# Go2Heart/StreamFormer

Hardware: AMD Instinct MI355X
Metric: frames/s (16x224^2 clips) (higher is better)
Workload: dtype bf16; 1 GPU; SigLIP-base StreamFormer encoder forward, 8 clips x 16 x 224^2 per GPU, random-init de-trivialised weights, causal temporal attention; global_batch_clips=8, frames_per_clip=16, parallelism=dp1, steps_in_flight=1

## Files before the change

include/streamformer_hip.h:

```cpp
#ifndef STREAMFORMER_HIP_H
#define STREAMFORMER_HIP_H

#include <stddef.h>
#include <stdint.h>

#ifdef __cplusplus
extern "C" {
#endif

typedef struct sf_encoder sf_encoder;
typedef struct sf_cache sf_cache;
typedef void* sf_stream;

typedef enum {
  SF_OK = 0,
  SF_ERR_INVALID = -1,
  SF_ERR_STATE = -2,
  SF_ERR_HIP = -3,
  SF_ERR_WORKSPACE = -4,
  SF_ERR_UNKNOWN_KEY = -5,
  SF_ERR_CAPACITY = -6
} sf_status;

typedef enum { SF_F32 = 0, SF_BF16 = 1, SF_F16 = 2, SF_F64 = 3, SF_U8 = 4 } sf_dtype;
// ... 72 lines not shown
  int32_t H, W;
  int32_t layers, hidden_size, patches;
  int32_t elem_bytes;
  uint64_t packing;
  uint64_t blob_bytes;
} sf_cache_stream_meta;
int sf_cache_stream_blob_bytes(const sf_cache* cache, int stream, size_t* out);
int sf_cache_export_stream(sf_encoder* enc, sf_cache* cache, int stream, void* blob_dev, size_t bytes,
                           sf_cache_stream_meta* meta_out, sf_stream s);
int sf_cache_import_stream(sf_encoder* enc, sf_cache* cache, int stream, const void* blob_dev, size_t bytes,
                           const sf_cache_stream_meta* meta, sf_stream s);

int sf_op_layernorm(const float* x_dev, const float* gamma_dev, const float* beta_dev, float* y_dev,
                    int rows, int D, float eps, sf_stream stream);
int sf_op_linear(const float* x_dev, const float* w_dev, const float* b_dev, const float* resid_dev,
                 float alpha, int gelu, float* y_dev, int M, int N, int K, int compute,
                 void* workspace_dev, size_t workspace_bytes, sf_stream stream);
size_t sf_op_linear_workspace_bytes(int M, int N, int K);
typedef struct {
  int32_t split;
  const uint16_t* a_hi; const uint16_t* a_lo;
  const uint16_t* w_hi; const uint16_t* w_lo;
  const float* bias;
  int32_t M, N, K, epi, act;
  float alpha;
  const float* resid; int32_t resid_mod;
  const uint16_t* resid_hi; const uint16_t* resid_lo; const uint16_t* resid_lo2;
  const float* pos; const float* time_rows; int32_t Np, Tn;
  float* out_f32; uint16_t* out_hi; uint16_t* out_lo; uint16_t* out_lo2; int32_t ldc;
  int32_t grp_rows, grp_stride, grp_off;
  float* ln_stats_out; const float* ln_stats; const float* ln_s; float ln_eps; int32_t ln_stats_wide, ln_inkernel;
} sf_gemm_desc;
int sf_op_gemm(const sf_gemm_desc* d, int family, int* family_taken, sf_stream stream);
int sf_op_attention(const float* qkv_dev, float* ctx_dev, int groups, int L, int heads, int head_dim,
                    int causal, int temporal_layout, int N_tokens, int compute,
                    void* workspace_dev, size_t workspace_bytes, sf_stream stream);
size_t sf_op_attention_workspace_bytes(int groups, int L, int heads, int head_dim);
typedef struct { int32_t stream, t_row, slot, tk; } sf_stream_slot;
int sf_op_attention_cached(const float* cache_dev, float* ctx_dev, int slabs, int cap, int N_tokens, int heads, int head_dim,
                           int compute, int B, int Tq, int Tk, int q_t0, int t_past, int causal, const int* pos_dev,
                           const sf_stream_slot* tab_dev, int* route_out, int* waves_out,
                           void* workspace_dev, size_t workspace_bytes, sf_stream stream);
size_t sf_op_attention_cached_workspace_bytes(int slabs, int cap, int N_tokens, int heads, int head_dim, int B, int Tq);

size_t sf_loss_workspace_bytes(int B, int T);
int sf_retrieval_loss(const float* pooler_dev, const float* text_dev, int B, int T, int D, int Bt,
                      int pos_offset, const float* logit_scale_dev, const float* logit_bias_dev,
                      float* loss_dev, float* grad_pooler_dev, float* grad_scalars_dev,
                      void* workspace_dev, size_t workspace_bytes, sf_stream stream);
int sf_localization_loss(const float* pooler_dev, const float* label_emb_dev, const int32_t* labels_dev,
                         int B, int T, int D, int L, const float* logit_scale_dev, const float* logit_bias_dev,
                         float* loss_dev, float* grad_pooler_dev, float* grad_scalars_dev,
                         void* workspace_dev, size_t workspace_bytes, sf_stream stream);

int sf_grounding_loss(const float* pooler_dev, const float* text_dev, const float* labels_dev, int B, int T, int D,
                      const float* logit_scale_dev, const float* logit_bias_dev, float* loss_dev, float* grad_pooler_dev,
                      float* grad_scalars_dev, float* logits_out_dev, void* workspace_dev, size_t workspace_bytes,
                      sf_stream stream);
int sf_dense_text_logits(const float* x_dev, const float* text_dev, int M, int D, int n, const float* logit_scale_dev,
                         const float* logit_bias_dev, float* out_dev, sf_stream stream);

size_t sf_mask_loss_workspace_bytes(int B, int T, int N, int L_max);
int sf_mask_loss(const float* x_dev, int B, int T, int N, int D, const float* const* label_emb_dev,
                 const int32_t* num_labels, const int32_t* const* mask_dev, const int32_t* mask_width, int H,
                 const float* logit_scale_dev, const float* logit_bias_dev, float* loss_dev, float* grad_x_dev,
                 float* grad_scalars_dev, void* workspace_dev, size_t workspace_bytes, sf_stream stream);
// ... 292 lines not shown
```

streamformer_amd/_native.py:

```python
from __future__ import annotations

import ctypes as C
import inspect
import os
import weakref

import torch

_HERE = os.path.dirname(os.path.abspath(__file__))
LIB_PATH = os.path.join(_HERE, "libstreamformer_hip.so")
if os.environ.get("SF_LIB"):
    LIB_PATH = os.path.join(_HERE, "libstreamformer_hip_%s.so" % os.environ["SF_LIB"])

SF_OK = 0
SF_ERR_INVALID, SF_ERR_STATE, SF_ERR_HIP, SF_ERR_WORKSPACE, SF_ERR_UNKNOWN_KEY, SF_ERR_CAPACITY = -1, -2, -3, -4, -5, -6
SF_F32, SF_BF16, SF_F16, SF_F64, SF_U8 = 0, 1, 2, 3, 4
SF_COMPUTE_BF16, SF_COMPUTE_BF16X3 = 0, 1


class SfConfig(C.Structure):
    _fields_ = [(n, C.c_int32) for n in (
        "image_size", "patch_size", "num_channels", "num_frames", "hidden_size", "num_hidden_layers",
        "num_attention_heads", "intermediate_size", "hidden_act", "qkv_bias", "enable_causal_temporal",
        "add_lora_spatial")] + [("layer_norm_eps", C.c_float)]
# ... 68 lines not shown
    "sf_destroy": (None, [_P]),
    "sf_last_error": (C.c_char_p, []),
    "sf_abi_version": (_I, []),
    "sf_load_tensor": (_I, [_P, C.c_char_p, _P, _I, C.POINTER(C.c_int64), _I]),
    "sf_finalize_weights": (_I, [_P, _I, _I, _I]),
    "sf_missing_weights": (_I, [_P]),
    "sf_set_pixel_normalization": (_I, [_P, _P, _P, _I, _F]),
    "sf_workspace_bytes": (_I, [_P, _I, _I, _I, _I, C.POINTER(_SZ)]),
    "sf_forward": (_I, [_P, _P, _I, _I, _I, _I, _I, _P, _P, _P, _P, _P, _SZ, _P]),
    "sf_forward_profile": (_I, [_P, _P, _I, _I, _I, _I, _I, _P, _P, _P, _SZ, _P, C.POINTER(_F)]),
    "sf_forward_attentions": (_I, [_P, _P, _I, _I, _I, _I, _I, _P, _P, _P, _P, _P, _P, _SZ, _P]),
    "sf_embed": (_I, [_P, _P, _I, _I, _I, _I, _I, _P, _P, _P, _SZ, _P]),
    "sf_layers": (_I, [_P, _P, _I, _I, _I, _I, _I, _I, _P, _P, _SZ, _P]),
    "sf_post_head": (_I, [_P, _P, _I, _I, _I, _I, _P, _P, _P, _SZ, _P]),
    "sf_cache_create": (_I, [_P, _I, _I, _I, _I, C.POINTER(_P)]),
    "sf_cache_reset": (_I, [_P]),
    "sf_cache_length": (_I, [_P]),
    "sf_cache_stream_length": (_I, [_P, _I]),
    "sf_cache_reset_stream": (_I, [_P, _I]),
    "sf_cache_bytes": (_SZ, [_P]),
    "sf_cache_set_policy": (_I, [_P, _I]),
    "sf_cache_destroy": (None, [_P]),
    "sf_cache_stream_blob_bytes": (_I, [_P, _I, C.POINTER(_SZ)]),
    "sf_cache_export_stream": (_I, [_P, _P, _I, _P, _SZ, C.POINTER(SfCacheStreamMeta), _P]),
    "sf_cache_import_stream": (_I, [_P, _P, _I, _P, _SZ, C.POINTER(SfCacheStreamMeta), _P]),
    "sf_stream_workspace_bytes": (_I, [_P, _P, _I, C.POINTER(_SZ)]),
    "sf_forward_stream": (_I, [_P, _P, _P, _I, _I, _P, _P, _P, _P, _P, _SZ, _P]),
    "sf_forward_stream_slots": (_I, [_P, _P, _P, _I, _I, C.POINTER(_I), _I, _P, _P, _P, _P, _SZ, _P]),
    "sf_forward_stream_attentions": (_I, [_P, _P, _P, _I, _I, _P, _P, _P, _P, _P, _P, _SZ, _P]),
    "sf_op_layernorm": (_I, [_P, _P, _P, _P, _I, _I, _F, _P]),
    "sf_op_linear": (_I, [_P, _P, _P, _P, _F, _I, _P, _I, _I, _I, _I, _P, _SZ, _P]),
    "sf_op_linear_workspace_bytes": (_SZ, [_I, _I, _I]),
    "sf_op_gemm": (_I, [C.POINTER(SfGemmDesc), _I, C.POINTER(_I), _P]),
    "sf_op_attention": (_I, [_P, _P, _I, _I, _I, _I, _I, _I, _I, _I, _P, _SZ, _P]),
    "sf_op_attention_workspace_bytes": (_SZ, [_I, _I, _I, _I]),
    "sf_op_attention_cached": (_I, [_P, _P, _I, _I, _I, _I, _I, _I, _I, _I, _I, _I, _I, _I, _P, _P, C.POINTER(_I), C.POINTER(_I), _P, _SZ, _P]),
    "sf_op_attention_cached_workspace_bytes": (_SZ, [_I, _I, _I, _I, _I, _I, _I]),
    "sf_loss_workspace_bytes": (_SZ, [_I, _I]),
    "sf_retrieval_loss": (_I, [_P, _P, _I, _I, _I, _I, _I, _P, _P, _P, _P, _P, _P, _SZ, _P]),
    "sf_localization_loss": (_I, [_P, _P, _P, _I, _I, _I, _I, _P, _P, _P, _P, _P, _P, _SZ, _P]),
    "sf_grounding_loss": (_I, [_P, _P, _P, _I, _I, _I, _P, _P, _P, _P, _P, _P, _P, _SZ, _P]),
    "sf_dense_text_logits": (_I, [_P, _P, _I, _I, _I, _P, _P, _P, _P]),
    "sf_mask_loss_workspace_bytes": (_SZ, [_I, _I, _I, _I]),
    "sf_mask_loss": (_I, [_P, _I, _I, _I, _I, C.POINTER(_P), C.POINTER(C.c_int32), C.POINTER(_P), C.POINTER(C.c_int32), _I,
                          _P, _P, _P, _P, _P, _P, _SZ, _P]),
    "sf_dense_head_workspace_bytes": (_SZ, [_I, _I, _I]),
    "sf_dense_head_forward": (_I, [_P, _I, _I, _I, _F, C.POINTER(_P), _P, _P, _SZ, _P]),
    "sf_dense_head_backward": (_I, [_P, _I, _I, _I, _F, C.POINTER(_P), _P, C.POINTER(_P), _P, _SZ, _P]),
    "sf_trainer_create": (_I, [C.POINTER(SfConfig), _I, _I, _I, C.POINTER(_P)]),
    "sf_trainer_destroy": (None, [_P]),
    "sf_trainer_num_params": (_I, [_P]),
    "sf_trainer_param_info": (_I, [_P, _I, C.c_char_p, _I, C.POINTER(C.c_int64), C.POINTER(C.c_int64),
                                   C.POINTER(C.c_int64), C.POINTER(_I), C.POINTER(_I), C.POINTER(_I)]),
    "sf_trainer_total_floats": (_I, [_P, C.POINTER(C.c_int64), C.POINTER(C.c_int64)]),
    "sf_trainer_num_stages": (_I, [_P]),
    "sf_trainer_stage_range": (_I, [_P, _I, C.POINTER(C.c_int64), C.POINTER(C.c_int64)]),
    "sf_trainer_sync_weights": (_I, [_P, _P, _P]),
    "sf_trainer_workspace_bytes": (_I, [_P, _I, _I, C.POINTER(_SZ)]),
    "sf_trainer_forward": (_I, [_P, _P, _I, _I, _I, _P, _P, _P, _SZ, _P]),
    "sf_trainer_backward": (_I, [_P, _P, _P, _P, _I, _I, _P, _SZ, _P]),
    "sf_trainer_adamw_step": (_I, [_P, _P, _P, _P, _P, _I, _F, _F, _F, _F, _F, _F, _P, _F, _I, _P]),
    "sf_trainer_set_drop_path": (_I, [_P, _P, _I, _I]),
    "sf_trainer_set_dropout": (_I, [_P, _F, _F, C.c_uint32]),
    "sf_trainer_set_nonfinite_guard": (_I, [_P, _P, _P]),
    "sf_trainer_set_extra_steps": (_I, [_P, C.POINTER(C.c_int32), _I]),
    "sf_trainer_grad_sumsq": (_I, [_P, _P, _P, _P]),
# ... 259 lines not shown
```

streamformer_amd/csrc/sf_common.h:

```cpp
#pragma once
#include <hip/hip_runtime.h>
#include <stdint.h>

typedef unsigned short bf16_t;

typedef __attribute__((ext_vector_type(8))) short bf16x8_t;
typedef __attribute__((ext_vector_type(4))) float f32x4_t;
typedef __attribute__((ext_vector_type(4))) unsigned int u32x4_t;
typedef __attribute__((ext_vector_type(2))) unsigned int u32x2_t;

#define SF_DEVICE __device__ __forceinline__

#ifdef SF_LAB
#define SF_LAB_SWITCH(name) (getenv(name) ? atoi(getenv(name)) : 0)
#else
#define SF_LAB_SWITCH(name) 0
#endif

SF_DEVICE int sf_swz64(int row) {
#ifdef SF_SWZ64_LEGACY
  return (row >> 2) & 3;
#else
  return (0 - (row >> 2)) & 3;
#endif
// ... 162 lines not shown

struct __attribute__((aligned(16))) SfStreamSlot { int stream, t_row, slot, tk; };
#define SF_MAX_CALL_STREAMS 64
struct SfStreamTable { int n; int pad[3]; SfStreamSlot e[SF_MAX_CALL_STREAMS]; };

struct SfGemmArgs {
  const bf16_t* a_hi; const bf16_t* a_lo;
  const bf16_t* w_hi; const bf16_t* w_lo;
  const float* bias;
  int M, N, K;
  int epi;
  int act;
  float alpha;
  const float* resid;
  int resid_mod;
  const bf16_t* resid_hi; const bf16_t* resid_lo;
  const bf16_t* resid_lo2; bf16_t* out_lo2;
  const float* pos; const float* time_rows;
  int Np, Tn;
  const int* time_base_dev;
  float* out_f32;
  bf16_t* out_hi; bf16_t* out_lo;
  int ldc;
  int grp_rows, grp_stride, grp_off;
  const int* grp_off_dev; int grp_off_scale;
  const SfStreamSlot* grp_tab;
  int w_nt;
  float* ln_stats_out;
  const float* ln_stats; const float* ln_s; float ln_eps;
  int ln_stats_wide;
  int ln_inkernel;
  int aux_mode;
  bf16_t* aux;
};
SF_DEVICE size_t sf_out_row(const SfGemmArgs& p, int m) {
  if (p.grp_rows <= 0) return (size_t)m;
  if (p.grp_tab) {
    const int g = m / p.grp_rows;
    const SfStreamSlot e = p.grp_tab[g];
    return (size_t)e.stream * p.grp_stride + e.slot * p.grp_off_scale + (m - g * p.grp_rows);
  }
  const int off = p.grp_off + (p.grp_off_dev ? *p.grp_off_dev * p.grp_off_scale : 0);
  return (size_t)(m / p.grp_rows) * p.grp_stride + off + (m % p.grp_rows);
}
int sf_wall_clock_ticks(int ns);
enum SfGemmFamily {
  SF_GEMM_FAM_NONE = 0,
  SF_GEMM_FAM_SKINNY = 1, SF_GEMM_FAM_TILE = 2, SF_GEMM_FAM_PANEL = 3, SF_GEMM_FAM_G256 = 4, SF_GEMM_FAM_G128 = 5,
  SF_GEMM_FAM_COLSPLIT = 6,
  SF_GEMM_FAM_LAB_PIPE = 7, SF_GEMM_FAM_LAB_PP = 8,
};
SfGemmFamily sf_gemm_family(const SfGemmArgs& a, bool split);
hipError_t sf_launch_gemm_family(SfGemmFamily fam, const SfGemmArgs& a, bool split, hipStream_t s);
hipError_t sf_launch_gemm(const SfGemmArgs& a, bool split, hipStream_t s);
bool sf_gemm128_supported(const SfGemmArgs& a, bool split);
hipError_t sf_launch_gemm128(const SfGemmArgs& a, bool split, hipStream_t s);
bool sf_gemm256_supported(const SfGemmArgs& a, bool split);
bool sf_gemm256_aux_supported(const SfGemmArgs& a);
hipError_t sf_launch_gemm256(const SfGemmArgs& a, hipStream_t s);
int sf_skinny_max_rows();
bool sf_gemm_skinny_supported(const SfGemmArgs& a, bool split);
hipError_t sf_launch_gemm_skinny(const SfGemmArgs& a, bool split, hipStream_t s);
bool sf_gemm_tile_supported(const SfGemmArgs& a, bool split);
hipError_t sf_launch_gemm_tile(const SfGemmArgs& a, hipStream_t s);
int sf_tile_max_rows();
int sf_tile_fold_min_rows();
int sf_infold_max_rows();
struct SfQkvArgs {
  const bf16_t* a;
  const bf16_t* w;
  const float* bias; const float* ln_s;
  const float* ln_stats; float ln_eps;
  int M, K, D;
  int B, T, NP;
  bf16_t* out;
  float scale; int causal;
};
bool sf_gemm_qkv_supported(const SfQkvArgs& a, bool fused);
hipError_t sf_launch_gemm_qkv(const SfQkvArgs& a, bool fused, hipStream_t s);
struct SfStreamQkvArgs {
  const bf16_t* a;
  const bf16_t* w_frag;
  const float* bias; const float* ln_s; float ln_eps;
  int M, K, D, heads, N;
  bf16_t* cache;
  int cap, slot, Tk;
  const int* pos_dev;
  bf16_t* ctx;
  float scale;
};
bool sf_stream_qkv_decode_supported(const SfStreamQkvArgs& a);
hipError_t sf_launch_stream_qkv_decode(const SfStreamQkvArgs& a, hipStream_t s);
// ... 117 lines not shown
```

streamformer_amd/csrc/sf_gemm256.hip:

```cpp
#include "sf_common.h"
#include "sf_switches.h"
#include <cstdlib>

#define G_THREADS 512
#define PIECE_BYTES 16384

typedef const __attribute__((address_space(1))) void* gptr_t;
typedef __attribute__((address_space(3))) void* lptr_t;

SF_DEVICE f32x4_t mfma16b(bf16x8_t a, bf16x8_t b, f32x4_t c) {
  typedef __attribute__((ext_vector_type(8))) __bf16 v8bf;
  return __builtin_amdgcn_mfma_f32_16x16x32_bf16(__builtin_bit_cast(v8bf, a), __builtin_bit_cast(v8bf, b), c, 0, 0, 0);
}

SF_DEVICE bf16x8_t rd_frag(const char* piece, int row, int kc) {
  return *reinterpret_cast<const bf16x8_t*>(piece + row * 128 + ((kc ^ ((row >> 1) & 7)) << 4));
}
SF_DEVICE bf16x8_t rd_frag_s(const char* piece, int plane, int row, int g) {
  return *reinterpret_cast<const bf16x8_t*>(piece + plane * 8192 + row * 64 + ((g ^ sf_swz64(row)) << 4));
}

#ifdef SF_G256_TRACE
__device__ unsigned long long g256_trace[16];
#endif

template <int N>
SF_DEVICE void wait_vm() {
  asm volatile("s_waitcnt vmcnt(%0)" ::"n"(N) : "memory");
}

#define G256_EPI_BF16_AUX 5

template <int EPI, bool LNF, int BM, bool SPLIT = false, bool WIDE = false>
__global__ __launch_bounds__(G_THREADS) void sf_gemm256_kernel(SfGemmArgs p, int ntiles, int stagger_ticks, int stagger_groups) {
  constexpr int HR = BM / 2;
  constexpr int MT1 = (HR - 64) / 16;
  extern __shared__ __attribute__((aligned(16))) char smem[];
  const int tid = threadIdx.x;
  const int lane = tid & 63;
  const int wave = __builtin_amdgcn_readfirstlane(tid >> 6);
  const int wm = wave >> 2, wn = wave & 3;
  const int l15 = lane & 15, g = lane >> 4;
  const int tiles_n = p.N >> 8;
  const int K = p.K;
  const int nkt = SPLIT ? (K >> 5) : (K >> 6);
  const int dma_lds = wave * 1024;
  const __amdgpu_buffer_rsrc_t rsrc_a = __builtin_amdgcn_make_buffer_rsrc((void*)p.a_hi, 0, (unsigned)p.M * (unsigned)K * 2u, 0x00020000);
  const __amdgpu_buffer_rsrc_t rsrc_w = __builtin_amdgcn_make_buffer_rsrc((void*)p.w_hi, 0, (unsigned)p.N * (unsigned)K * 2u, 0x00020000);
  const __amdgpu_buffer_rsrc_t rsrc_al = __builtin_amdgcn_make_buffer_rsrc((void*)(SPLIT ? p.a_lo : p.a_hi), 0, (unsigned)p.M * (unsigned)K * 2u, 0x00020000);
  const __amdgpu_buffer_rsrc_t rsrc_wl = __builtin_amdgcn_make_buffer_rsrc((void*)(SPLIT ? p.w_lo : p.w_hi), 0, (unsigned)p.N * (unsigned)K * 2u, 0x00020000);
  const int cpx = gridDim.x >> 3;
  const int xcd = blockIdx.x & 7, slot_in_xcd = blockIdx.x >> 3;
  const int walk_cg = (stagger_groups >> 8) & 15;
  const bool store_wt = (stagger_groups >> 12) & 1;
  const bool store_nt = (stagger_groups >> 13) & 1;
  stagger_groups &= 255;
  const int walk_ngrp = walk_cg ? (tiles_n + walk_cg - 1) / walk_cg : 1;
  const int walk_per = (ntiles + 7) >> 3;
  const int walk_panels = ntiles / tiles_n;

  if (stagger_ticks > 0) {
    const int grp = slot_in_xcd % stagger_groups;
    if (grp) {
      const unsigned long long t0 = wall_clock64();
      const unsigned long long wait = (unsigned long long)grp * (unsigned long long)stagger_ticks;
      while (wall_clock64() - t0 < wait) __builtin_amdgcn_s_sleep(8);
    }
  }

#ifdef SF_G256_TRACE
  unsigned tr_read = 0, tr_bar1 = 0, tr_mma = 0, tr_bar2 = 0;
#endif
  for (int round = 0;; ++round) {
#ifdef SF_G256_TRACE
    tr_read = tr_bar1 = tr_mma = tr_bar2 = 0;
#endif
    int tile = (round * 8 + xcd) * cpx + slot_in_xcd;
    int m0, n0;
    if (walk_cg == 15) {
      const int sg = stagger_groups, grp = slot_in_xcd % sg, ig = slot_in_xcd / sg;
      const int n_g = (cpx - grp + sg - 1) / sg;
      const int before = grp * (cpx / sg) + min(grp, cpx % sg);
      const int x0 = xcd * walk_per, x1 = min(x0 + walk_per, ntiles);
      const int lo = x0 + (int)((long)(x1 - x0) * before / cpx), hi = x0 + (int)((long)(x1 - x0) * (before + n_g) / cpx);
      tile = lo + round * n_g + ig;
      if (tile >= hi) break;
      m0 = (tile / tiles_n) * BM; n0 = (tile % tiles_n) << 8;
    } else if (walk_cg) {
      const int tloc = round * cpx + slot_in_xcd;
      tile = xcd * walk_per + tloc;
      if (tloc >= walk_per || tile >= ntiles) break;
      int rest = tile, c0 = 0, w = 0;
      for (int j = 0; j < walk_ngrp; ++j) {
        w = tiles_n / walk_ngrp + (j < tiles_n % walk_ngrp ? 1 : 0);
        if (rest < walk_panels * w) break;
        rest -= walk_panels * w; c0 += w;
      }
      m0 = (rest / w) * BM; n0 = (c0 + rest % w) << 8;
    } else {
      if (tile >= ntiles) break;
      m0 = (tile / tiles_n) * BM; n0 = (tile % tiles_n) << 8;
    }

    unsigned offA[2][2], offB[2][2];
    int tid_p = threadIdx.x;
    asm volatile("" : "+v"(tid_p));
#pragma unroll
    for (int i = 0; i < (SPLIT ? 1 : 2); ++i) {
      const int c = i * G_THREADS + tid_p;
      const int prow = SPLIT ? (c >> 2) : (c >> 3), slot = SPLIT ? (c & 3) : (c & 7);
      const int kc = SPLIT ? (slot ^ sf_swz64(prow)) : (slot ^ ((prow >> 1) & 7));
#pragma unroll
      for (int q = 0; q < 2; ++q) {
        int rr = prow & 63;
        if (q == 1 && rr >= MT1 * 16) rr = MT1 * 16 - 1;
        int ar = m0 + (prow >> 6) * HR + q * 64 + rr;
        ar = ar < p.M ? ar : p.M - 1;
        offA[q][i] = ((unsigned)ar * (unsigned)K + kc * 8) * 2u;
        int br = n0 + (prow >> 5) * 64 + q * 32 + (prow & 31);
        offB[q][i] = ((unsigned)br * (unsigned)K + kc * 8) * 2u;
      }
    }
    auto issue = [&](int t, int j) {
      char* dst = smem + ((t & 1) * 4 + j) * PIECE_BYTES + dma_lds;
      const unsigned o0 = (j & 1) ? offA[j >> 1][0] : offB[j >> 1][0];
      const unsigned o1 = (j & 1) ? offA[j >> 1][SPLIT ? 0 : 1] : offB[j >> 1][SPLIT ? 0 : 1];
      const int kof = SPLIT ? t * 64 : t * 128;
      if (SPLIT) {
        if (j & 1) {
          __builtin_amdgcn_raw_ptr_buffer_load_lds(rsrc_a, (lptr_t)dst, 16, o0, kof, 0, 0);
          __builtin_amdgcn_raw_ptr_buffer_load_lds(rsrc_al, (lptr_t)(dst + 8192), 16, o1, kof, 0, 0);
        } else {
// ... 347 lines not shown
  if (split && a.ln_stats && (!a.ln_stats_wide || !a.ln_s || (a.K % 256) || a.K > 1024 || (a.epi != SF_EPI_BF16 && a.epi != SF_EPI_ACT_BF16))) return false;
  if (a.epi == SF_EPI_EMBED_F32) return false;
  bool planes = false;
  if (a.epi == SF_EPI_RESID_F32 && a.out_hi) {
    if (!a.out_lo || !a.resid_hi || !a.resid_lo || !a.ln_stats_out || !a.ln_stats_wide || (a.N % 256) || a.N > 1024 || a.grp_rows > 0) return false;
    if (!split && (a.resid_lo2 || a.out_lo2)) return false;
    planes = true;
  } else if (a.resid_hi) {
    return false;
  }
  if (!split && a.epi == SF_EPI_ACT_BF16 && a.act != 0 && a.act != 99) return false;
  if (a.K % 128 || a.K < 128) return false;
  int min_n = 1024;
  if (split) {
    min_n = a.M <= 6272 ? 1024 : 768;
    if (const char* e = sf_sw(SW_G256_SPLIT_MIN_N)) min_n = atoi(e);
  }
  if (a.N % 256 || a.N < min_n) return false;
  if (a.M < 2048 || (size_t)a.M * a.K * 2 >= ((size_t)1 << 32) || (size_t)a.N * a.K * 2 >= ((size_t)1 << 32)) return false;
  if (a.out_lo && !split && !planes) return false;
  return true;
}

bool sf_gemm256_aux_supported(const SfGemmArgs& a) {
  return a.epi == SF_EPI_BF16 && a.aux != nullptr && sf_gemm256_supported(a, false);
}

static int g256_grid() {
  int cus = sf_device_cus();
  if (cus < 8) cus = 256;
  return cus & ~7;
}

template <int BM, bool SPLIT_ONLY = false>
static hipError_t launch_bm(const SfGemmArgs& a_in, hipStream_t s) {
  SfGemmArgs a = a_in;
  if (SF_LAB_SWITCH("SF_G256_LAB_NOSTORE")) a.act = 99;
  const int tiles = ((a.M + BM - 1) / BM) * (a.N / 256);
  const size_t lds = 8 * PIECE_BYTES;
  const dim3 grid(g256_grid()), block(G_THREADS);
  int stagger = 0, sgroups = 3;
  if (const char* ge = sf_sw(SW_G256_STAGGER_GROUPS)) sgroups = atoi(ge) > 1 ? atoi(ge) : 2;
  {
    const int rounds = (tiles + (int)grid.x - 1) / (int)grid.x;
    double pct = 21.0;
    if (const char* pe = sf_sw(SW_G256_STAGGER_PCT)) pct = atof(pe);
    const char* env = sf_sw(SW_G256_STAGGER_NS);
    if (env) stagger = sf_wall_clock_ticks(atoi(env));
    else if (rounds >= 3) {
      const double mfma_x = (a.a_lo && a.w_lo) ? 3.0 : 1.0;
      const double tile_ns = mfma_x * 2.0 * BM * 256.0 * a.K / 3.9e3 + 6500.0;
      stagger = sf_wall_clock_ticks((int)(tile_ns * pct / 100.0));
    }
  }
  if (const char* only = sf_sw(SW_G256_STAGGER_ONLY)) {
    if (a.epi != atoi(only)) stagger = 0;
  }
  {
    int cg = 0;
    if (const char* we = sf_sw(SW_G256_WALK)) cg = atoi(we);
    if (cg < 0 || cg > 15 || (cg != 15 && cg >= a.N / 256)) cg = 0;
    sgroups = (sgroups & 255) | (cg << 8) | (sf_sw(SW_G256_STORE_WT) ? 1 << 12 : 0) | (sf_sw(SW_G256_STORE_NT) ? 1 << 13 : 0);
  }
#define SF_LAUNCH256(E, L, SP) return sf_launch_big_lds(sf_gemm256_kernel<E, L, BM, SP>, grid, block, lds, s, a, tiles, stagger, sgroups)
  if (a.a_lo && a.w_lo) {
    if (a.aux_mode) return hipErrorInvalidValue;
    if (a.ln_stats) {
      if (!a.ln_stats_wide || !a.ln_s) return hipErrorInvalidValue;
      if (a.epi == SF_EPI_BF16) SF_LAUNCH256(SF_EPI_BF16, true, true);
      if (a.epi == SF_EPI_ACT_BF16) SF_LAUNCH256(SF_EPI_ACT_BF16, true, true);
      return hipErrorInvalidValue;
    }
    switch (a.epi) {
#define SF_CASE(E) case E: SF_LAUNCH256(E, false, true);
      SF_CASE(SF_EPI_F32) SF_CASE(SF_EPI_BF16) SF_CASE(SF_EPI_ACT_BF16) SF_CASE(SF_EPI_RESID_F32)
#undef SF_CASE
      default: return hipErrorInvalidValue;
    }
  }
  if constexpr (SPLIT_ONLY) return hipErrorInvalidValue;
  else {
  const bool lnf = a.ln_stats != nullptr;
  if (lnf && (!a.ln_s || (a.epi != SF_EPI_BF16 && a.epi != SF_EPI_ACT_BF16))) return hipErrorInvalidValue;
  switch (a.epi) {
    case SF_EPI_F32: SF_LAUNCH256(SF_EPI_F32, false, false);
    case SF_EPI_BF16:
      if (a.aux_mode) {
        if (lnf || !a.aux) return hipErrorInvalidValue;
        SF_LAUNCH256(G256_EPI_BF16_AUX, false, false);
      }
      if (lnf) SF_LAUNCH256(SF_EPI_BF16, true, false);
      SF_LAUNCH256(SF_EPI_BF16, false, false);
    case SF_EPI_ACT_BF16:
      if (lnf) SF_LAUNCH256(SF_EPI_ACT_BF16, true, false);
      SF_LAUNCH256(SF_EPI_ACT_BF16, false, false);
    case SF_EPI_RESID_F32: SF_LAUNCH256(SF_EPI_RESID_F32, false, false);
    default: return hipErrorInvalidValue;
  }
  }
#undef SF_LAUNCH256
}

hipError_t sf_launch_gemm256(const SfGemmArgs& a, hipStream_t s) {
  const int g = g256_grid(), nt = a.N / 256;
  auto cost = [&](int bm) { const int tiles = ((a.M + bm - 1) / bm) * nt; return (long)((tiles + g - 1) / g) * bm; };
  if (a.a_lo && a.w_lo && !sf_sw(SW_G256_NO_SHORT_BM)) {
    auto t = [&](int bm, double f) { return (double)cost(bm) / bm * f; };
    const double t256 = t(256, 1632), t224 = t(224, 1472), t192 = t(192, 1370), t160 = t(160, 1268);
    const double best = fmin(fmin(t256, t224), fmin(t192, t160));
    if (const char* fe = sf_sw(SW_G256_FORCE_BM)) {
      switch (atoi(fe)) { case 160: return launch_bm<160, true>(a, s); case 192: return launch_bm<192, true>(a, s); case 224: return launch_bm<224>(a, s); default: return launch_bm<256>(a, s); }
    }
    if (best == t160 && t160 < 0.97 * fmin(t224, t256)) return launch_bm<160, true>(a, s);
    if (best == t192 && t192 < 0.97 * fmin(t224, t256)) return launch_bm<192, true>(a, s);
  }
  if (cost(224) < cost(256) && !sf_sw(SW_G256_NO_BM224)) return launch_bm<224>(a, s);
  return launch_bm<256>(a, s);
}
```

streamformer_amd/csrc/sf_ops.hip:

```cpp
#include "sf_handle.h"

#include <cmath>
#include <cstring>

__global__ void sf_combine_kernel(const bf16_t* hi, const bf16_t* lo, float* out, size_t n) {
  for (size_t i = (size_t)blockIdx.x * blockDim.x + threadIdx.x; i < n; i += (size_t)gridDim.x * blockDim.x)
    out[i] = bf2f(hi[i]) + (lo ? bf2f(lo[i]) : 0.f);
}

extern "C" int sf_op_layernorm(const float* x, const float* gamma, const float* beta, float* y, int rows, int D,
                               float eps, sf_stream stream) {
  HIP_TRY(sf_launch_layernorm(x, gamma, beta, y, nullptr, nullptr, rows, D, eps, (hipStream_t)stream));
  return SF_OK;
}

extern "C" size_t sf_op_linear_workspace_bytes(int M, int N, int K) {
  return ((size_t)M * K * 2 + (size_t)N * K * 2 + (size_t)M * N * 2) * 2 + 4096;
}

extern "C" int sf_op_linear(const float* x, const float* w, const float* b, const float* resid, float alpha, int gelu,
                            float* y, int M, int N, int K, int compute, void* workspace, size_t workspace_bytes,
                            sf_stream stream) {
  if (workspace_bytes < sf_op_linear_workspace_bytes(M, N, K)) return sf_set_err(SF_ERR_WORKSPACE, "workspace too small");
  hipStream_t s = (hipStream_t)stream;
  const bool split = compute == SF_COMPUTE_BF16X3;
  SfCarver c(workspace, split, true);
  const SfPlanes xp = c.planes((size_t)M * K), wp = c.planes((size_t)N * K), op = c.planes((size_t)M * N);
  HIP_TRY(sf_launch_split(x, xp.hi, xp.lo, (size_t)M * K, s));
  HIP_TRY(sf_launch_split(w, wp.hi, wp.lo, (size_t)N * K, s));
  SfGemmArgs g;
  memset(&g, 0, sizeof(g));
  g.a_hi = xp.hi; g.a_lo = xp.lo; g.w_hi = wp.hi; g.w_lo = wp.lo; g.bias = b;
  g.M = M; g.N = N; g.K = K; g.ldc = N; g.alpha = alpha; g.resid = resid; g.act = 0;
  if (gelu) {
    g.epi = SF_EPI_ACT_BF16; g.out_hi = op.hi; g.out_lo = op.lo;
    HIP_TRY(sf_launch_gemm(g, split, s));
    HIP_TRY(sf_launch(sf_combine_kernel, dim3(1024), dim3(256), 0, s, op.hi, op.lo, y, (size_t)M * N));
  } else {
    g.epi = resid ? SF_EPI_RESID_F32 : SF_EPI_F32; g.out_f32 = y;
    HIP_TRY(sf_launch_gemm(g, split, s));
  }
  return SF_OK;
}

static const char* gemm_family_name(int f) {
  static const char* const names[] = {"none", "skinny", "tile", "panel", "256^2", "128^2", "256-column + 128-column tail", "lab pipe", "lab pp"};
  return f >= 0 && f <= 8 ? names[f] : "?";
}
extern "C" int sf_op_gemm(const sf_gemm_desc* d, int family, int* family_taken, sf_stream stream) {
  if (family_taken) *family_taken = SF_GEMM_FAM_NONE;
  if (!d) return sf_set_err(SF_ERR_INVALID, "sf_op_gemm: null descriptor");
  if (family < 0 || family > SF_GEMM_FAM_G128) return sf_set_err(SF_ERR_INVALID, "sf_op_gemm: family %d is not one of 0 (dispatch) .. 5", family);
  const bool split = d->split != 0;
  if (d->M <= 0 || d->N <= 0 || d->K <= 0) return sf_set_err(SF_ERR_INVALID, "sf_op_gemm: bad shape M=%d N=%d K=%d", d->M, d->N, d->K);
  if (d->ldc < d->N) return sf_set_err(SF_ERR_INVALID, "sf_op_gemm: ldc %d < N %d", d->ldc, d->N);
  if (!d->a_hi || !d->w_hi) return sf_set_err(SF_ERR_INVALID, "sf_op_gemm: a_hi and w_hi are required");
  if (split && (!d->a_lo || !d->w_lo)) return sf_set_err(SF_ERR_INVALID, "sf_op_gemm: split needs a_lo and w_lo");
  if (!split && (d->a_lo || d->w_lo)) return sf_set_err(SF_ERR_INVALID, "sf_op_gemm: a_lo / w_lo given without split");
  if (d->act < 0 || d->act > 2) return sf_set_err(SF_ERR_INVALID, "sf_op_gemm: act %d is not 0 (erf GELU), 1 (tanh GELU) or 2 (ReLU)", d->act);
  if (d->resid_mod < 0) return sf_set_err(SF_ERR_INVALID, "sf_op_gemm: resid_mod %d < 0", d->resid_mod);
  if (d->resid_mod > 0 && !d->resid) return sf_set_err(SF_ERR_INVALID, "sf_op_gemm: resid_mod needs the fp32 resid table");
  if ((d->resid_hi != nullptr) != (d->resid_lo != nullptr)) return sf_set_err(SF_ERR_INVALID, "sf_op_gemm: resid_hi and resid_lo come together");
  if (d->resid_lo2 && !d->resid_hi) return sf_set_err(SF_ERR_INVALID, "sf_op_gemm: resid_lo2 needs resid_hi and resid_lo");
  if (d->resid && d->resid_hi) return sf_set_err(SF_ERR_INVALID, "sf_op_gemm: resid and resid_hi / resid_lo are two forms of one operand: give one");
  if (d->out_lo && !d->out_hi) return sf_set_err(SF_ERR_INVALID, "sf_op_gemm: out_lo needs out_hi");
  if (d->out_lo2 && !d->out_lo) return sf_set_err(SF_ERR_INVALID, "sf_op_gemm: out_lo2 needs out_hi and out_lo");
  if (!d->ln_inkernel && (d->ln_stats != nullptr) != (d->ln_s != nullptr))
    return sf_set_err(SF_ERR_INVALID, "sf_op_gemm: ln_stats and ln_s come together");
  if (d->ln_inkernel && !d->ln_s) return sf_set_err(SF_ERR_INVALID, "sf_op_gemm: ln_inkernel needs ln_s");
  if (d->ln_inkernel && d->ln_stats) return sf_set_err(SF_ERR_INVALID, "sf_op_gemm: ln_inkernel and ln_stats are two forms of one fold: give one");
  if ((d->ln_stats || d->ln_inkernel) && d->ln_stats_out) return sf_set_err(SF_ERR_INVALID, "sf_op_gemm: a fold consumer does not produce statistics");
  if (d->grp_rows < 0 || (d->grp_rows > 0 && (d->grp_stride < d->grp_rows || d->grp_off < 0)))
    return sf_set_err(SF_ERR_INVALID, "sf_op_gemm: row remap grp_rows=%d grp_stride=%d grp_off=%d (stride >= rows > 0, off >= 0)", d->grp_rows, d->grp_stride, d->grp_off);
  switch (d->epi) {
// ... 187 lines not shown
```

streamformer_amd/csrc/sf_switches.h:

```cpp
#pragma once

#define SF_SWITCH_TABLE(X) \
  X(ACC_TWO_PLANES, "SF_ACC_TWO_PLANES", "accurate mode: residual stream as two planes instead of three (A/B; max-abs 1.4e-4 instead of 5e-5)") \
  X(ASSUME_CUS, "SF_ASSUME_CUS", "size persistent grids for this many CUs (CU-masked stream experiments)") \
  X(DISABLE_ACC_FOLD, "SF_DISABLE_ACC_FOLD", "accurate mode: fp32 residual + standalone LayerNorm instead of the folded plane form (A/B)") \
  X(DISABLE_G256_SPLIT, "SF_DISABLE_G256_SPLIT", "accurate mode: keep the bf16x3 GEMMs off the persistent 256-column kernel") \
  X(DISABLE_GEMM_COLSPLIT, "SF_DISABLE_GEMM_COLSPLIT", "N = 256 j + 128 (so400m widths): the whole GEMM on 128^2 tiles instead of 256-column kernel + a 128-column tail (A/B)") \
  X(DISABLE_GEMM_MID, "SF_DISABLE_GEMM_MID", "skinny family: no 64 x 64 tiles above 512 rows") \
  X(DISABLE_GEMM_TILE, "SF_DISABLE_GEMM_TILE", "one / two clips per call: no tile-GEMM family") \
  X(DISABLE_LN_FOLD, "SF_DISABLE_LN_FOLD", "bf16 mode: standalone LayerNorm launches instead of the fold into the consumer GEMMs (A/B)") \
  X(DISABLE_RESID_PLANES, "SF_DISABLE_RESID_PLANES", "bf16 mode: fp32 residual stream instead of hi + lo planes (A/B)") \
  X(DISABLE_SKG_UNROLL, "SF_DISABLE_SKG_UNROLL", "streaming: K-parallel skinny GEMM with a run-time K-tile count (A/B)") \
  X(DISABLE_SKINNY, "SF_DISABLE_SKINNY", "send small-M GEMMs to the generic 128^2 kernel") \
  X(DISABLE_SPATIAL_DMA, "SF_DISABLE_SPATIAL_DMA", "spatial attention on the register-staged kernel") \
  X(DISABLE_SPATIAL_DMA_ACC, "SF_DISABLE_SPATIAL_DMA_ACC", "accurate mode: spatial attention on fp32 q / k / v (test coverage of that path)") \
  X(DISABLE_SPATIAL_NTC, "SF_DISABLE_SPATIAL_NTC", "spatial attention with a run-time tile count (A/B)") \
  X(DISABLE_STREAM_FOLD, "SF_DISABLE_STREAM_FOLD", "streaming: standalone LayerNorm launches (A/B)") \
  X(DISABLE_STREAM_GRAPH, "SF_DISABLE_STREAM_GRAPH", "streaming: eager launches instead of hipGraph replay") \
  X(DISABLE_TEMPORAL_DECODE, "SF_DISABLE_TEMPORAL_DECODE", "streaming: general temporal kernel instead of the single-query one") \
  X(TBWD_OWN_CU, "SF_TBWD_OWN_CU", "training: temporal attention backward as 12-wave workgroups that own a CU instead of 4-wave workgroups with their exact LDS (bit-identical, 65 against 51 us per launch; for jobs that share a device, DESIGN.md 4)") \
  X(TEMPORAL_DECODE_LANE_KEY, "SF_TEMPORAL_DECODE_LANE_KEY", "streaming: single-query temporal kernel with one key per lane (A/B against whole-line loads)") \
  X(DISABLE_TEMPORAL_DMA, "SF_DISABLE_TEMPORAL_DMA", "temporal attention on the register-staged kernel") \
  X(DISABLE_TEMPORAL_DMA_ACC, "SF_DISABLE_TEMPORAL_DMA_ACC", "accurate mode: temporal attention on fp32 q / k / v (test coverage of that path)") \
  X(EMBED_VIA_GEMM128, "SF_EMBED_VIA_GEMM128", "embedding GEMM on the generic kernel (A/B)") \
  X(G256_FORCE_BM, "SF_G256_FORCE_BM", "256-column kernel: force the row-tile height (tests of the short tiles)") \
  X(G256_NO_BM224, "SF_G256_NO_BM224", "256-column kernel: no 224-row tiles") \
  X(G256_NO_SHORT_BM, "SF_G256_NO_SHORT_BM", "256-column kernel, accurate mode: no 160 / 192-row tiles") \
  X(G256_SPLIT_MIN_N, "SF_G256_SPLIT_MIN_N", "accurate mode: smallest N the persistent kernel takes") \
  X(G256_WALK, "SF_G256_WALK", "256-column kernel: column-group width (tiles) of the column-group-major tile walk, 0 = row-major (A/B of the fabric traffic)") \
  X(G256_STORE_WT, "SF_G256_STORE_WT", "256-column kernel: bf16 outputs leave with write-through (sc1) stores that do not stay in the XCD's L2 (A/B)") \
  X(G256_STORE_NT, "SF_G256_STORE_NT", "256-column kernel: bf16 outputs leave with non-temporal stores (A/B: do the residual planes then survive in the Infinity Cache?)") \
  X(G256_STAGGER_GROUPS, "SF_G256_STAGGER_GROUPS", "256-column kernel: phase-stagger groups per XCD") \
  X(G256_STAGGER_NS, "SF_G256_STAGGER_NS", "256-column kernel: stagger step in ns (overrides the percentage)") \
  X(G256_STAGGER_ONLY, "SF_G256_STAGGER_ONLY", "256-column kernel: stagger only some launches (A/B)") \
  X(G256_STAGGER_PCT, "SF_G256_STAGGER_PCT", "256-column kernel: stagger step as a percentage of the tile period") \
  X(GEMM_MID_MIN_M, "SF_GEMM_MID_MIN_M", "skinny family: first M of the 64 x 64 tiles") \
  X(LN_BWD_BLOCKS, "SF_LN_BWD_BLOCKS", "LayerNorm backward: workgroups (tuning)") \
  X(POOL_SHARE_CU, "SF_POOL_SHARE_CU", "pooling head: the probe / combine kernels request only the LDS they use instead of a CU's whole 160 KB (A/B; with it other workgroups share their CUs, see DESIGN.md 4 on device sharing)") \
  X(PANEL_MIN_FILL_PCT, "SF_PANEL_MIN_FILL_PCT", "panel kernel: minimum last-round fill") \
  X(PANEL_PAD_CLAMP, "SF_PANEL_PAD_CLAMP", "panel kernel: clamp instead of zero-fill the padding rows (A/B)") \
  X(PANEL_STAGGER_NS, "SF_PANEL_STAGGER_NS", "panel kernel: phase-stagger step in ns") \
  X(SKINNY_MAX_M, "SF_SKINNY_MAX_M", "skinny family: largest M") \
  X(SKINNY_NO_KG, "SF_SKINNY_NO_KG", "skinny family: no K-parallel variant") \
  X(SKINNY_NB, "SF_SKINNY_NB", "streaming, folded skinny consumers: 1 = 32 x 32 tiles everywhere, 2 / 3 = force 32 x 64 / 32 x 96 tiles (A/B)") \
  X(SKINNY_NT, "SF_SKINNY_NT", "skinny family: non-temporal weight loads (A/B)") \
  X(SKINNY_TPS, "SF_SKINNY_TPS", "skinny family: tiles per slot (tuning)") \
  X(SPATIAL_PERS, "SF_SPATIAL_PERS", "lab library: persistent spatial attention kernel") \
  X(SPATIAL_TPW, "SF_SPATIAL_TPW", "spatial attention: query tiles per workgroup (tuning)") \
  X(STREAM_GRAPH_PER_POSITION, "SF_STREAM_GRAPH_PER_POSITION", "streaming: one graph per cache position instead of the position-free one (A/B)") \
  X(TILE_FOLD_MIN_M, "SF_TILE_FOLD_MIN_M", "tile-GEMM family: smallest M whose LayerNorm fold uses a statistics buffer and the 256^2 consumers") \
  X(TILE_MAX_M, "SF_TILE_MAX_M", "tile-GEMM family: largest M") \
  X(TILE_MIN_M, "SF_TILE_MIN_M", "tile-GEMM family: smallest M") \
  X(TILE_SHAPE, "SF_TILE_SHAPE", "tile-GEMM family: force a tile shape (tools/tile_lab.py)") \
  X(TRAIN_UNFUSED_TEMPORAL, "SF_TRAIN_UNFUSED_TEMPORAL", "training: temporal_attention.output.dense and temporal_dense as two launches instead of one fused projection (A/B)") \
  X(TRAIN_SIDE_STREAM, "SF_TRAIN_SIDE_STREAM", "training: 0 keeps the LoRA gradients on the caller stream (A/B)") \
  X(WGRAD_NSPLIT, "SF_WGRAD_NSPLIT", "weight-gradient GEMM: force the token splits") \
  X(WGRAD_SMALL_TILES, "SF_WGRAD_SMALL_TILES", "weight-gradient GEMM: 128^2 tiles only") \
  X(WGRAD_UNGROUPED, "SF_WGRAD_UNGROUPED", "training: one weight-gradient launch per projection instead of one per layer (test / A/B)") \

enum SfSw {
#define SF_SW_ENUM(id, name, what) SW_##id,
  SF_SWITCH_TABLE(SF_SW_ENUM)
// ... 5 lines not shown
```

Before: 15780 frames/s.

## Plan tail-round tile split across phase-staggered groups in the 256-column GEMM

Adds a host-side run planner that sizes each stagger group's tile share by when that group starts, so early-starting groups take more tail tiles and later groups fewer, rather than splitting in proportion to slot counts. The persistent 256-column kernel reads the planned group boundaries and, in the row-major walk, hands out last-round tiles per group from them. The aim is to shorten the tail left idle by the phase stagger. The cost is extra index arithmetic in the kernel and a planner whose timing model (tile period, step fraction) may not match the hardware.

```diff
diff --git a/include/streamformer_hip.h b/include/streamformer_hip.h
--- a/include/streamformer_hip.h
+++ b/include/streamformer_hip.h
@@ -128,6 +128,8 @@
   float* ln_stats_out; const float* ln_stats; const float* ln_s; float ln_eps; int32_t ln_stats_wide, ln_inkernel;
 } sf_gemm_desc;
 int sf_op_gemm(const sf_gemm_desc* d, int family, int* family_taken, sf_stream stream);
+int sf_g256_plan_runs(int tiles, int slots, int groups, double step, int* counts, double* ends);
+int sf_g256_launch_plan(int M, int N, int K, int split, int* out, double* ends);
 int sf_op_attention(const float* qkv_dev, float* ctx_dev, int groups, int L, int heads, int head_dim,
                     int causal, int temporal_layout, int N_tokens, int compute,
                     void* workspace_dev, size_t workspace_bytes, sf_stream stream);
diff --git a/streamformer_amd/_native.py b/streamformer_amd/_native.py
--- a/streamformer_amd/_native.py
+++ b/streamformer_amd/_native.py
@@ -124,6 +124,8 @@
     "sf_op_linear": (_I, [_P, _P, _P, _P, _F, _I, _P, _I, _I, _I, _I, _P, _SZ, _P]),
     "sf_op_linear_workspace_bytes": (_SZ, [_I, _I, _I]),
     "sf_op_gemm": (_I, [C.POINTER(SfGemmDesc), _I, C.POINTER(_I), _P]),
+    "sf_g256_plan_runs": (_I, [_I, _I, _I, C.c_double, C.POINTER(_I), C.POINTER(C.c_double)]),
+    "sf_g256_launch_plan": (_I, [_I, _I, _I, _I, C.POINTER(_I), C.POINTER(C.c_double)]),
     "sf_op_attention": (_I, [_P, _P, _I, _I, _I, _I, _I, _I, _I, _I, _P, _SZ, _P]),
     "sf_op_attention_workspace_bytes": (_SZ, [_I, _I, _I, _I]),
     "sf_op_attention_cached": (_I, [_P, _P, _I, _I, _I, _I, _I, _I, _I, _I, _I, _I, _I, _I, _P, _P, C.POINTER(_I), C.POINTER(_I), _P, _SZ, _P]),
diff --git a/streamformer_amd/csrc/sf_common.h b/streamformer_amd/csrc/sf_common.h
--- a/streamformer_amd/csrc/sf_common.h
+++ b/streamformer_amd/csrc/sf_common.h
@@ -218,6 +218,7 @@
   int ln_inkernel;
   int aux_mode;
   bf16_t* aux;
+  int g256_b1, g256_b2;
 };
 SF_DEVICE size_t sf_out_row(const SfGemmArgs& p, int m) {
   if (p.grp_rows <= 0) return (size_t)m;
@@ -244,6 +245,7 @@
 bool sf_gemm256_supported(const SfGemmArgs& a, bool split);
 bool sf_gemm256_aux_supported(const SfGemmArgs& a);
 hipError_t sf_launch_gemm256(const SfGemmArgs& a, hipStream_t s);
+void sf_gemm256_launch_plan(int M, int N, int K, bool split, int* out, double* ends);
 int sf_skinny_max_rows();
 bool sf_gemm_skinny_supported(const SfGemmArgs& a, bool split);
 hipError_t sf_launch_gemm_skinny(const SfGemmArgs& a, bool split, hipStream_t s);
diff --git a/streamformer_amd/csrc/sf_g256_plan.h b/streamformer_amd/csrc/sf_g256_plan.h
--- /dev/null
+++ b/streamformer_amd/csrc/sf_g256_plan.h
@@ -0,0 +1,82 @@
+#pragma once
+
+#define SF_G256_PLAN_MAX_GROUPS 8
+
+struct SfG256RunPlan {
+  int count[SF_G256_PLAN_MAX_GROUPS];
+  int slots[SF_G256_PLAN_MAX_GROUPS];
+  double end;
+  double end_proportional;
+  int weighted;
+};
+
+static inline int sf_g256_slots_before(int slots, int groups, int g) { return g * (slots / groups) + (g < slots % groups ? g : slots % groups); }
+
+static inline int sf_g256_proportional_bound(int tiles, int slots, int groups, int g) {
+  return (int)((long long)tiles * sf_g256_slots_before(slots, groups, g) / slots);
+}
+
+static inline double sf_g256_plan_end(const int* count, const int* slots, int groups, double step) {
+  double end = 0.0;
+  for (int g = 0; g < groups; ++g) {
+    if (count[g] <= 0) continue;
+    const double e = g * step + (double)((count[g] + slots[g] - 1) / slots[g]);
+    if (e > end) end = e;
+  }
+  return end;
+}
+
+static inline bool sf_g256_plan_group_runs(int tiles, int slots, int groups, double step, SfG256RunPlan* plan) {
+  if (tiles < 0 || slots < 1 || groups < 2 || groups > SF_G256_PLAN_MAX_GROUPS || groups > slots || !(step >= 0.0)) return false;
+  int prop[SF_G256_PLAN_MAX_GROUPS];
+  for (int g = 0; g < groups; ++g) {
+    plan->slots[g] = sf_g256_slots_before(slots, groups, g + 1) - sf_g256_slots_before(slots, groups, g);
+    prop[g] = sf_g256_proportional_bound(tiles, slots, groups, g + 1) - sf_g256_proportional_bound(tiles, slots, groups, g);
+  }
+  plan->end_proportional = sf_g256_plan_end(prop, plan->slots, groups, step);
+  const double eps = 1e-9;
+  const int max_rounds = (tiles + plan->slots[groups - 1] - 1) / plan->slots[groups - 1] + 1;
+  double best = -1.0;
+  for (int gc = 0; gc < groups; ++gc)
+    for (int r = 0; r <= max_rounds; ++r) {
+      const double e = gc * step + r;
+      if (best >= 0.0 && e >= best - eps) break;
+      long long cap = 0;
+      for (int g = 0; g < groups; ++g) {
+        const double room = e - g * step + eps;
+        if (room >= 1.0) cap += (long long)plan->slots[g] * (long long)room;
+      }
+      if (cap >= tiles) { best = e; break; }
+    }
+  if (best < 0.0 || best >= plan->end_proportional - eps) {
+    for (int g = 0; g < groups; ++g) plan->count[g] = prop[g];
+    plan->end = plan->end_proportional;
+    plan->weighted = 0;
+    return true;
+  }
+  long long slack = -(long long)tiles;
+  int rounds[SF_G256_PLAN_MAX_GROUPS];
+  for (int g = 0; g < groups; ++g) {
+    const double room = best - g * step + eps;
+    rounds[g] = room >= 1.0 ? (int)room : 0;
+    plan->count[g] = plan->slots[g] * rounds[g];
+    slack += plan->count[g];
+  }
+  while (slack > 0) {
+    int last = -1;
+    double last_end = -1.0;
+    for (int g = 0; g < groups; ++g) {
+      if (plan->count[g] <= 0) continue;
+      const double e = g * step + (double)((plan->count[g] + plan->slots[g] - 1) / plan->slots[g]);
+      if (e > last_end + eps) { last_end = e; last = g; }
+    }
+    const int spare = (plan->count[last] - 1) % plan->slots[last];
+    long long take = spare > 0 ? spare : 1;
+    if (take > slack) take = slack;
+    plan->count[last] -= (int)take;
+    slack -= take;
+  }
+  plan->end = sf_g256_plan_end(plan->count, plan->slots, groups, step);
+  plan->weighted = 1;
+  return true;
+}
diff --git a/streamformer_amd/csrc/sf_gemm256.hip b/streamformer_amd/csrc/sf_gemm256.hip
--- a/streamformer_amd/csrc/sf_gemm256.hip
+++ b/streamformer_amd/csrc/sf_gemm256.hip
@@ -1,5 +1,6 @@
 #include "sf_common.h"
 #include "sf_switches.h"
+#include "sf_g256_plan.h"
 #include <cstdlib>
 
 #define G_THREADS 512
@@ -54,6 +55,7 @@
   const int walk_cg = (stagger_groups >> 8) & 15;
   const bool store_wt = (stagger_groups >> 12) & 1;
   const bool store_nt = (stagger_groups >> 13) & 1;
+  const bool run_plan = (stagger_groups >> 14) & 1;
   stagger_groups &= 255;
   const int walk_ngrp = walk_cg ? (tiles_n + walk_cg - 1) / walk_cg : 1;
   const int walk_per = (ntiles + 7) >> 3;
@@ -82,7 +84,13 @@
       const int n_g = (cpx - grp + sg - 1) / sg;
       const int before = grp * (cpx / sg) + min(grp, cpx % sg);
       const int x0 = xcd * walk_per, x1 = min(x0 + walk_per, ntiles);
-      const int lo = x0 + (int)((long)(x1 - x0) * before / cpx), hi = x0 + (int)((long)(x1 - x0) * (before + n_g) / cpx);
+      int lo, hi;
+      if (run_plan) {
+        lo = min(x0 + (grp == 0 ? 0 : grp == 1 ? p.g256_b1 : p.g256_b2), x1);
+        hi = min(x0 + (grp == 0 ? p.g256_b1 : grp == 1 ? p.g256_b2 : walk_per), x1);
+      } else {
+        lo = x0 + (int)((long)(x1 - x0) * before / cpx); hi = x0 + (int)((long)(x1 - x0) * (before + n_g) / cpx);
+      }
       tile = lo + round * n_g + ig;
       if (tile >= hi) break;
       m0 = (tile / tiles_n) * BM; n0 = (tile % tiles_n) << 8;
@@ -98,6 +106,18 @@
       }
       m0 = (rest / w) * BM; n0 = (c0 + rest % w) << 8;
     } else {
+      const int full = ntiles / (int)gridDim.x;
+      if (run_plan && round >= full) {
+        int slot_p = slot_in_xcd;
+        asm volatile("" : "+s"(slot_p));
+        const int sg = stagger_groups, grp = slot_p % sg, ig = slot_p / sg;
+        const int n_g = (cpx - grp + sg - 1) / sg;
+        const int rest = ntiles - full * (int)gridDim.x, part = (rest + 7) >> 3;
+        const int lo = grp == 0 ? 0 : grp == 1 ? p.g256_b1 : p.g256_b2, hi = grp == 0 ? p.g256_b1 : grp == 1 ? p.g256_b2 : part;
+        const int j = lo + (round - full) * n_g + ig;
+        if (j >= hi || xcd * part + j >= rest) break;
+        tile = full * (int)gridDim.x + xcd * part + j;
+      }
       if (tile >= ntiles) break;
       m0 = (tile / tiles_n) * BM; n0 = (tile % tiles_n) << 8;
     }
@@ -511,6 +531,65 @@
   return cus & ~7;
 }
 
+struct SfG256Schedule {
+  int stagger;
+  int packed;
+  int b1, b2;
+  int planned;
+  double end, end_before;
+};
+
+static SfG256Schedule sf_g256_schedule(const SfGemmArgs& a, int BM, int tiles, int grid) {
+  SfG256Schedule sch = {};
+  int stagger = 0, sgroups = 3;
+  if (const char* ge = sf_sw(SW_G256_STAGGER_GROUPS)) sgroups = atoi(ge) > 1 ? atoi(ge) : 2;
+  const int rounds = (tiles + grid - 1) / grid;
+  const double mfma_x = (a.a_lo && a.w_lo) ? 3.0 : 1.0;
+  const double tile_ns = mfma_x * 2.0 * BM * 256.0 * a.K / 3.9e3 + 6500.0;
+  int step_ns = 0;
+  {
+    double pct = 21.0;
+    if (const char* pe = sf_sw(SW_G256_STAGGER_PCT)) pct = atof(pe);
+    if (const char* env = sf_sw(SW_G256_STAGGER_NS)) step_ns = atoi(env);
+    else if (rounds >= 3) step_ns = (int)(tile_ns * pct / 100.0);
+    if (step_ns) stagger = sf_wall_clock_ticks(step_ns);
+  }
+  if (const char* only = sf_sw(SW_G256_STAGGER_ONLY)) {
+    if (a.epi != atoi(only)) stagger = 0;
+  }
+  int cg = 0;
+  bool plan_off = false;
+  if (const char* we = sf_sw(SW_G256_WALK)) {
+    cg = atoi(we);
+    if (cg < 0) { plan_off = true; cg = cg == -15 ? 15 : 0; }
+  }
+  if (cg > 15 || (cg != 15 && cg >= a.N / 256)) cg = 0;
+  const int cpx = grid >> 3;
+  if (stagger > 0 && rounds >= 3 && sgroups == 3 && cpx >= 3 && (cg == 0 || cg == 15)) {
+    const double step = (double)step_ns / tile_ns;
+    SfG256RunPlan plan;
+    if (cg == 15) {
+      const int per = (tiles + 7) >> 3;
+      if (sf_g256_plan_group_runs(per, cpx, 3, step, &plan)) {
+        sch.end = plan.end; sch.end_before = plan.end_proportional;
+        if (plan_off) sch.end = sch.end_before;
+        else if (plan.weighted) { sch.planned = 1; sch.b1 = plan.count[0]; sch.b2 = plan.count[0] + plan.count[1]; }
+      }
+    } else {
+      const int full = tiles / grid, rest = tiles - full * grid, part = (rest + 7) >> 3;
+      const int busy = rest < cpx ? rest : cpx;
+      sch.end = sch.end_before = rest ? full + 1 + ((busy < 3 ? busy : 3) - 1) * step : full + 2 * step;
+      if (rest && !plan_off && sf_g256_plan_group_runs(full * cpx + part, cpx, 3, step, &plan) && plan.weighted && plan.end < sch.end_before - 1e-9) {
+        const int e0 = plan.count[0] - full * plan.slots[0], e1 = plan.count[1] - full * plan.slots[1], e2 = plan.count[2] - full * plan.slots[2];
+        if (e0 >= 0 && e1 >= 0 && e2 >= 0) { sch.planned = 1; sch.b1 = e0; sch.b2 = e0 + e1; sch.end = plan.end; }
+      }
+    }
+  }
+  sch.stagger = stagger;
+  sch.packed = (sgroups & 255) | (cg << 8) | (sf_sw(SW_G256_STORE_WT) ? 1 << 12 : 0) | (sf_sw(SW_G256_STORE_NT) ? 1 << 13 : 0) | (sch.planned << 14);
+  return sch;
+}
+
 template <int BM, bool SPLIT_ONLY = false>
 static hipError_t launch_bm(const SfGemmArgs& a_in, hipStream_t s) {
   SfGemmArgs a = a_in;
@@ -518,29 +597,9 @@
   const int tiles = ((a.M + BM - 1) / BM) * (a.N / 256);
   const size_t lds = 8 * PIECE_BYTES;
   const dim3 grid(g256_grid()), block(G_THREADS);
-  int stagger = 0, sgroups = 3;
-  if (const char* ge = sf_sw(SW_G256_STAGGER_GROUPS)) sgroups = atoi(ge) > 1 ? atoi(ge) : 2;
-  {
-    const int rounds = (tiles + (int)grid.x - 1) / (int)grid.x;
-    double pct = 21.0;
-    if (const char* pe = sf_sw(SW_G256_STAGGER_PCT)) pct = atof(pe);
-    const char* env = sf_sw(SW_G256_STAGGER_NS);
-    if (env) stagger = sf_wall_clock_ticks(atoi(env));
-    else if (rounds >= 3) {
-      const double mfma_x = (a.a_lo && a.w_lo) ? 3.0 : 1.0;
-      const double tile_ns = mfma_x * 2.0 * BM * 256.0 * a.K / 3.9e3 + 6500.0;
-      stagger = sf_wall_clock_ticks((int)(tile_ns * pct / 100.0));
-    }
-  }
-  if (const char* only = sf_sw(SW_G256_STAGGER_ONLY)) {
-    if (a.epi != atoi(only)) stagger = 0;
-  }
-  {
-    int cg = 0;
-    if (const char* we = sf_sw(SW_G256_WALK)) cg = atoi(we);
-    if (cg < 0 || cg > 15 || (cg != 15 && cg >= a.N / 256)) cg = 0;
-    sgroups = (sgroups & 255) | (cg << 8) | (sf_sw(SW_G256_STORE_WT) ? 1 << 12 : 0) | (sf_sw(SW_G256_STORE_NT) ? 1 << 13 : 0);
-  }
+  const SfG256Schedule sch = sf_g256_schedule(a, BM, tiles, (int)grid.x);
+  const int stagger = sch.stagger, sgroups = sch.packed;
+  a.g256_b1 = sch.b1; a.g256_b2 = sch.b2;
 #define SF_LAUNCH256(E, L, SP) return sf_launch_big_lds(sf_gemm256_kernel<E, L, BM, SP>, grid, block, lds, s, a, tiles, stagger, sgroups)
   if (a.a_lo && a.w_lo) {
     if (a.aux_mode) return hipErrorInvalidValue;
@@ -580,7 +639,7 @@
 #undef SF_LAUNCH256
 }
 
-hipError_t sf_launch_gemm256(const SfGemmArgs& a, hipStream_t s) {
+static int g256_row_tile(const SfGemmArgs& a) {
   const int g = g256_grid(), nt = a.N / 256;
   auto cost = [&](int bm) { const int tiles = ((a.M + bm - 1) / bm) * nt; return (long)((tiles + g - 1) / g) * bm; };
   if (a.a_lo && a.w_lo && !sf_sw(SW_G256_NO_SHORT_BM)) {
@@ -588,11 +647,32 @@
     const double t256 = t(256, 1632), t224 = t(224, 1472), t192 = t(192, 1370), t160 = t(160, 1268);
     const double best = fmin(fmin(t256, t224), fmin(t192, t160));
     if (const char* fe = sf_sw(SW_G256_FORCE_BM)) {
-      switch (atoi(fe)) { case 160: return launch_bm<160, true>(a, s); case 192: return launch_bm<192, true>(a, s); case 224: return launch_bm<224>(a, s); default: return launch_bm<256>(a, s); }
-    }
-    if (best == t160 && t160 < 0.97 * fmin(t224, t256)) return launch_bm<160, true>(a, s);
-    if (best == t192 && t192 < 0.97 * fmin(t224, t256)) return launch_bm<192, true>(a, s);
-  }
-  if (cost(224) < cost(256) && !sf_sw(SW_G256_NO_BM224)) return launch_bm<224>(a, s);
-  return launch_bm<256>(a, s);
-}
+      switch (atoi(fe)) { case 160: return 160; case 192: return 192; case 224: return 224; default: return 256; }
+    }
+    if (best == t160 && t160 < 0.97 * fmin(t224, t256)) return 160;
+    if (best == t192 && t192 < 0.97 * fmin(t224, t256)) return 192;
+  }
+  if (cost(224) < cost(256) && !sf_sw(SW_G256_NO_BM224)) return 224;
+  return 256;
+}
+
+hipError_t sf_launch_gemm256(const SfGemmArgs& a, hipStream_t s) {
+  switch (g256_row_tile(a)) {
+    case 160: return launch_bm<160, true>(a, s);
+    case 192: return launch_bm<192, true>(a, s);
+    case 224: return launch_bm<224>(a, s);
+    default: return launch_bm<256>(a, s);
+  }
+}
+
+void sf_gemm256_launch_plan(int M, int N, int K, bool split, int* out, double* ends) {
+  SfGemmArgs a = {};
+  a.M = M; a.N = N; a.K = K;
+  static const bf16_t mark = 0;
+  if (split) a.a_lo = a.w_lo = &mark;
+  const int bm = g256_row_tile(a), grid = g256_grid(), tiles = ((M + bm - 1) / bm) * (N / 256);
+  const SfG256Schedule sch = sf_g256_schedule(a, bm, tiles, grid);
+  const int vals[10] = {bm, grid, tiles, sch.stagger, sch.packed & 255, (sch.packed >> 8) & 15, sch.planned, sch.b1, sch.b2, tiles / grid};
+  for (int i = 0; i < 10; ++i) out[i] = vals[i];
+  if (ends) { ends[0] = sch.end; ends[1] = sch.end_before; }
+}
diff --git a/streamformer_amd/csrc/sf_ops.hip b/streamformer_amd/csrc/sf_ops.hip
--- a/streamformer_amd/csrc/sf_ops.hip
+++ b/streamformer_amd/csrc/sf_ops.hip
@@ -1,4 +1,5 @@
 #include "sf_handle.h"
+#include "sf_g256_plan.h"
 
 #include <cmath>
 #include <cstring>
@@ -40,6 +41,20 @@
     g.epi = resid ? SF_EPI_RESID_F32 : SF_EPI_F32; g.out_f32 = y;
     HIP_TRY(sf_launch_gemm(g, split, s));
   }
+  return SF_OK;
+}
+
+extern "C" int sf_g256_plan_runs(int tiles, int slots, int groups, double step, int* counts, double* ends) {
+  SfG256RunPlan plan;
+  if (!counts || !sf_g256_plan_group_runs(tiles, slots, groups, step, &plan))
+    return sf_set_err(SF_ERR_INVALID, "sf_g256_plan_runs: tiles=%d slots=%d groups=%d step=%g (2 <= groups <= %d, groups <= slots, step >= 0)", tiles, slots, groups, step, SF_G256_PLAN_MAX_GROUPS);
+  for (int g = 0; g < groups; ++g) counts[g] = plan.count[g];
+  if (ends) { ends[0] = plan.end; ends[1] = plan.end_proportional; }
+  return SF_OK;
+}
+extern "C" int sf_g256_launch_plan(int M, int N, int K, int split, int* out, double* ends) {
+  if (M <= 0 || N < 256 || (N % 256) || K <= 0 || !out) return sf_set_err(SF_ERR_INVALID, "sf_g256_launch_plan: bad shape M=%d N=%d K=%d, or no output array", M, N, K);
+  sf_gemm256_launch_plan(M, N, K, split != 0, out, ends);
   return SF_OK;
 }
 
diff --git a/streamformer_amd/csrc/sf_switches.h b/streamformer_amd/csrc/sf_switches.h
--- a/streamformer_amd/csrc/sf_switches.h
+++ b/streamformer_amd/csrc/sf_switches.h
@@ -27,7 +27,7 @@
   X(G256_NO_BM224, "SF_G256_NO_BM224", "256-column kernel: no 224-row tiles") \
   X(G256_NO_SHORT_BM, "SF_G256_NO_SHORT_BM", "256-column kernel, accurate mode: no 160 / 192-row tiles") \
   X(G256_SPLIT_MIN_N, "SF_G256_SPLIT_MIN_N", "accurate mode: smallest N the persistent kernel takes") \
-  X(G256_WALK, "SF_G256_WALK", "256-column kernel: column-group width (tiles) of the column-group-major tile walk, 0 = row-major (A/B of the fabric traffic)") \
+  X(G256_WALK, "SF_G256_WALK", "256-column kernel: column-group width (tiles) of the column-group-major tile walk, 0 = row-major, 15 = row-major with one run per stagger group (A/B of the fabric traffic); negative = the stagger groups' runs without the run plan, every group a share in proportion to its slots: -1 row-major, -15 one run per group (A/B of the plan)") \
   X(G256_STORE_WT, "SF_G256_STORE_WT", "256-column kernel: bf16 outputs leave with write-through (sc1) stores that do not stay in the XCD's L2 (A/B)") \
   X(G256_STORE_NT, "SF_G256_STORE_NT", "256-column kernel: bf16 outputs leave with non-temporal stores (A/B: do the residual planes then survive in the Infinity Cache?)") \
   X(G256_STAGGER_GROUPS, "SF_G256_STAGGER_GROUPS", "256-column kernel: phase-stagger groups per XCD") \
```

Result: no change. 15890 frames/s, median of 6 (+0.7%).
